# Xharlie/BtcDet

Hardware: AMD Instinct MI355X
Metric: scenes/s fwd+bwd KITTI-Car bs=2/GPU (BtcDet hot path) (higher is better)
Workload: dtype f32

## Files before the change

### btcdet_amd/_lib.py

```python
import ctypes
import os

import numpy as np
import torch

_HERE = os.path.dirname(os.path.abspath(__file__))
LIB_PATH = os.path.join(_HERE, "libbtcdet_hip.so")
_lib = None

c_i32p = ctypes.POINTER(ctypes.c_int32)
c_f32p = ctypes.POINTER(ctypes.c_float)
vp = ctypes.c_void_p
ci = ctypes.c_int
sz = ctypes.c_size_t

MODE_SUBM, MODE_CONV, MODE_TRANSPOSE = 0, 1, 2


class BtcHipError(RuntimeError):
    pass


class BtcOccConfig(ctypes.Structure):
    _fields_ = [("batch", ctypes.c_int32), ("grid", ctypes.c_int32 * 3), ("sphere_grid", ctypes.c_int32 * 3),
# ... 169 lines not shown

AUGMENT_EXPORTED_SYMBOLS = tuple(_AUGMENT_SIGS.keys())

_BESTMATCH_SIGS = {
    "btc_place_templates": (ci, [vp, ctypes.c_longlong, vp, vp, vp, vp, vp, ci, ci, vp, vp, ctypes.c_longlong, ci, vp, vp]),
}

BESTMATCH_EXPORTED_SYMBOLS = tuple(_BESTMATCH_SIGS.keys())

_FRAMES_SIGS = {
    "btc_fov_crop_ws_bytes": (sz, [ci, ci]),
    "btc_fov_crop": (ci, [vp, ci, ci, vp, ci, vp, ci, vp, vp, vp, vp, sz, vp]),
}

FRAMES_EXPORTED_SYMBOLS = tuple(_FRAMES_SIGS.keys())

_GTDB_SIGS = {
    "btc_cut_objects_ws_bytes": (sz, [ci, ci, ci, ci]),
    "btc_cut_objects": (ci, [vp, ci, ci, vp, ci, vp, vp, vp, ci, ci, ci, vp, vp, vp, vp, sz, vp]),
}

GTDB_EXPORTED_SYMBOLS = tuple(_GTDB_SIGS.keys())

cf = ctypes.c_float
_TEMPLATES_SIGS = {
    "btc_nn_sqdist": (ci, [vp, ci, vp, ci, vp, vp, ci, ci, vp, vp]),
    "btc_match_candidates": (ci, [vp, ci, vp, vp, ci, vp, vp, ci, ci, cf, cf, cf, ci, ci, vp, vp, vp]),
    "btc_select_templates_ws_bytes": (sz, [ci, ci, ci]),
    "btc_select_templates": (ci, [vp, ci, vp, ci, vp, vp, vp, vp, vp, vp, ci, ci, ci, ci, ci, cf, cf, cf, ci, ci, vp, vp, vp, vp, vp, sz, vp]),
}

TEMPLATES_EXPORTED_SYMBOLS = tuple(_TEMPLATES_SIGS.keys())


def lib():
    global _lib
    if _lib is None:
        if not os.path.exists(LIB_PATH):
            raise BtcHipError(
                f"{LIB_PATH} not found: build it with `python -c 'import __graft_entry__ as g; g.build()'` "
                f"or `make -C btcdet_amd/csrc` (there is no CPU fallback for the hot path)")
        L = ctypes.CDLL(LIB_PATH)
        for name, (res, args) in (list(_SIGS.items()) + list(_INFER_SIGS.items()) + list(_AUGMENT_SIGS.items()) + list(_BESTMATCH_SIGS.items()) +
                                  list(_FRAMES_SIGS.items()) + list(_GTDB_SIGS.items()) + list(_TEMPLATES_SIGS.items())):
            fn = getattr(L, name)
            fn.restype = res
            fn.argtypes = args
        for kv in filter(None, os.environ.get("BTC_TUNE", "").split(",")):
            k, v = kv.split("=")
            if L.btc_tune_set(int(k), int(v)) != 0:
                raise BtcHipError("BTC_TUNE: bad entry %r" % kv)
        _lib = L
    return _lib


_fast = False


def fast():
    global _fast
    if _fast is False:
        _fast = None
        if os.environ.get("BTC_FASTPATH", "1") != "0":
            try:
                lib()
                from . import _btcfast
                if _btcfast.abi_version() == lib().btc_version():
                    _fast = _btcfast
            except ImportError:
                _fast = None
    return _fast


def check(rc, what):
    if rc != 0:
        msg = lib().btc_last_error().decode("utf-8", "replace")
        raise BtcHipError(f"{what} failed (code {rc}): {msg}")
# ... 55 lines not shown
```

### btcdet_amd/csrc/binding.cpp

```cpp
#include <torch/extension.h>
#include <c10/hip/HIPCachingAllocator.h>
#include <c10/hip/HIPStream.h>
#include <c10/hip/HIPGuard.h>
#include <hip/hip_runtime_api.h>
#include <torch/csrc/autograd/engine.h>

#include <atomic>
#include <mutex>
#include <stdexcept>
#include <string>
#include <unordered_map>
#include <cstdio>
#include <cstdlib>
#include <memory>
#include <tuple>
#include <vector>

#include "../../include/btcdet_hip.h"
#include "../../include/btcdet_hip_infer.h"

namespace {

using at::Tensor;
using OptTensor = c10::optional<at::Tensor>;

inline void chk(int rc, const char* what) {
  if (rc != 0) throw std::runtime_error(std::string(what) + " failed (code " + std::to_string(rc) + "): " + btc_last_error());
}

inline const float* fptr(const OptTensor& t) { return (t.has_value() && t->defined()) ? (const float*)t->data_ptr() : nullptr; }
inline void* vptr(const OptTensor& t) { return (t.has_value() && t->defined()) ? t->data_ptr() : nullptr; }
inline void* st(int64_t stream) { return reinterpret_cast<void*>(stream); }
inline const int32_t* ip(int64_t p) { return reinterpret_cast<const int32_t*>(p); }


inline void need(bool ok, const char* msg) {
  if (!ok) throw std::runtime_error(msg);
}
inline void need(bool ok, const char* who, const char* msg) {
  if (!ok) throw std::runtime_error(std::string(who) + msg);
}

struct WqEntry {
  c10::weak_intrusive_ptr<c10::TensorImpl> weak;
  uint32_t version;
  Tensor q;
  WqEntry(c10::weak_intrusive_ptr<c10::TensorImpl> w, uint32_t v, Tensor t) : weak(std::move(w)), version(v), q(std::move(t)) {}
};
std::mutex g_wq_mu;
std::unordered_map<const void*, WqEntry> g_wq;
std::unordered_map<const void*, WqEntry> g_ws;

// ... 793 lines not shown
    }
    x = ConvBNReLUNode::apply(x, weights[i], biases[i], map_fwd[i], map_bwd[i], order_fwd[i], order_bwd[i], gammas[i], betas[i], rms[i], rvs[i], nbts[i], use_batch[i],
                              momenta[i], epss[i], relus[i], ws, ws_bytes[i], overlaps[i], allow_defers[i]);
  }
  return x;
}

void adam_group_step(const std::vector<Tensor>& params, const std::vector<Tensor>& grads, const Tensor& chunk_seg, const Tensor& chunk_off,
                     const Tensor& chunk_len, const Tensor& chunk_flat, const std::vector<int64_t>& seg_chunk0, const Tensor& flat_p,
                     const Tensor& flat_m, const Tensor& flat_v, int64_t step, double lr, double beta1, double beta2, double eps, double weight_decay,
                     double clip, const Tensor& ws, int64_t stream) {
  const size_t n = params.size();
  need(grads.size() == n && seg_chunk0.size() == n + 1, "adam_group_step: list lengths differ");
  std::vector<const float*> ptrs(n);
  std::vector<int32_t> sc(n + 1);
  for (size_t i = 0; i < n; ++i) {
    const Tensor& g = grads[i];
    need(g.defined() && g.is_contiguous() && g.scalar_type() == at::kFloat && g.numel() == params[i].numel() && g.get_device() == flat_p.get_device(),
         "adam_group_step: every gradient must be a contiguous fp32 tensor of its parameter's size on the parameters' device");
    ptrs[i] = (const float*)g.data_ptr();
    sc[i] = (int32_t)seg_chunk0[i];
  }
  sc[n] = (int32_t)seg_chunk0[n];
  chk(btc_adam_group_step(ptrs.data(), (int)n, (const int32_t*)chunk_seg.data_ptr(), (const int32_t*)chunk_off.data_ptr(),
                          (const int32_t*)chunk_len.data_ptr(), (const int64_t*)chunk_flat.data_ptr(), sc.data(), (int)chunk_seg.numel(),
                          (float*)flat_p.data_ptr(), (float*)flat_m.data_ptr(), (float*)flat_v.data_ptr(), (long long)step, (float)lr, (float)beta1,
                          (float)beta2, (float)eps, (float)weight_decay, (float)clip, ws.data_ptr(), (size_t)ws.numel(), st(stream)),
      "btc_adam_group_step");
  for (size_t i = 0; i < n; ++i) params[i].unsafeGetTensorImpl()->bump_version();
}

struct ParamList {
  std::vector<Tensor> p;
};

std::shared_ptr<ParamList> make_param_list(const std::vector<Tensor>& params) {
  auto pl = std::make_shared<ParamList>();
  pl->p = params;
  return pl;
}

bool adam_group_step_pl(const std::shared_ptr<ParamList>& pl, const Tensor& chunk_seg, const Tensor& chunk_off, const Tensor& chunk_len,
                        const Tensor& chunk_flat, const std::vector<int64_t>& seg_chunk0, const Tensor& flat_p, const Tensor& flat_m,
                        const Tensor& flat_v, int64_t step, double lr, double beta1, double beta2, double eps, double weight_decay, double clip,
                        const Tensor& ws, int64_t stream) {
  const size_t n = pl->p.size();
  std::vector<Tensor> grads(n);
  for (size_t i = 0; i < n; ++i) {
    const Tensor& g = pl->p[i].grad();
    if (!(g.defined() && g.is_contiguous() && g.scalar_type() == at::kFloat && g.numel() == pl->p[i].numel() && g.get_device() == flat_p.get_device()))
      return false;
    grads[i] = g;
  }
  adam_group_step(pl->p, grads, chunk_seg, chunk_off, chunk_len, chunk_flat, seg_chunk0, flat_p, flat_m, flat_v, step, lr, beta1, beta2, eps,
                  weight_decay, clip, ws, stream);
  return true;
}

void clear_grads_pl(const std::shared_ptr<ParamList>& pl) {
  for (Tensor& t : pl->p) t.mutable_grad().reset();
}

void pack_grads(const std::vector<Tensor>& grads, const Tensor& chunk_seg, const Tensor& chunk_off, const Tensor& chunk_len, const Tensor& chunk_flat,
                const std::vector<int64_t>& seg_chunk0, const std::vector<int64_t>& sizes, const Tensor& flat, int64_t stream) {
  const size_t n = grads.size();
  need(seg_chunk0.size() == n + 1 && sizes.size() == n, "pack_grads: list lengths differ");
  std::vector<const float*> ptrs(n);
  std::vector<int32_t> sc(n + 1);
  for (size_t i = 0; i < n; ++i) {
    const Tensor& g = grads[i];
    need(g.defined() && g.is_contiguous() && g.scalar_type() == at::kFloat && g.numel() == sizes[i] && g.get_device() == flat.get_device(),
         "pack_grads: every gradient must be a contiguous fp32 tensor of its parameter's size on the bucket's device");
    ptrs[i] = (const float*)g.data_ptr();
    sc[i] = (int32_t)seg_chunk0[i];
  }
  sc[n] = (int32_t)seg_chunk0[n];
  chk(btc_grads_pack(ptrs.data(), (int)n, (const int32_t*)chunk_seg.data_ptr(), (const int32_t*)chunk_off.data_ptr(), (const int32_t*)chunk_len.data_ptr(),
                     (const int64_t*)chunk_flat.data_ptr(), sc.data(), (float*)flat.data_ptr(), st(stream)), "btc_grads_pack");
}

}

PYBIND11_MODULE(TORCH_EXTENSION_NAME, m) {
  m.doc() = "compiled PyTorch binding of libbtcdet_hip.so's hot entry points";
  m.def("split_weights", &split_weights, py::call_guard<py::gil_scoped_release>());
  m.def("bf16_weights", &bf16_weights, py::call_guard<py::gil_scoped_release>());
  m.def("conv_fwd", &conv_fwd, py::call_guard<py::gil_scoped_release>());
  m.def("bn_fwd", &bn_fwd, py::call_guard<py::gil_scoped_release>());
  m.def("conv_bn_fwd", &conv_bn_fwd, py::call_guard<py::gil_scoped_release>());
  m.def("conv_bn_eval_fold", &conv_bn_eval_fold, py::call_guard<py::gil_scoped_release>());
  m.def("eval_fold_calls", &eval_fold_calls);
  m.def("bn_bwd", &bn_bwd, py::call_guard<py::gil_scoped_release>());
  m.def("conv_bwd", &conv_bwd, py::call_guard<py::gil_scoped_release>());
  m.def("conv_bn_relu", &conv_bn_relu, py::call_guard<py::gil_scoped_release>());
  m.def("row_orders", &row_orders, py::call_guard<py::gil_scoped_release>());
  m.def("geometry_walk", &geometry_walk, py::call_guard<py::gil_scoped_release>());
  py::class_<PendingWalk, std::shared_ptr<PendingWalk>>(m, "PendingWalk");
  m.def("geometry_walk_start", &geometry_walk_start, py::call_guard<py::gil_scoped_release>());
  m.def("geometry_walk_finish", &geometry_walk_finish, py::call_guard<py::gil_scoped_release>());
  m.def("conv_bn_relu_chain", &conv_bn_relu_chain, py::call_guard<py::gil_scoped_release>());
  m.def("pack_grads", &pack_grads, py::call_guard<py::gil_scoped_release>());
  m.def("adam_group_step", &adam_group_step, py::call_guard<py::gil_scoped_release>());
  py::class_<ParamList, std::shared_ptr<ParamList>>(m, "ParamList");
  m.def("make_param_list", &make_param_list);
  m.def("adam_group_step_pl", &adam_group_step_pl, py::call_guard<py::gil_scoped_release>());
  m.def("clear_grads_pl", &clear_grads_pl);
  m.def("join_wgrad", &join_wgrad, py::call_guard<py::gil_scoped_release>());
  m.def("set_defer_wgrad_join", &set_defer_wgrad_join);
  m.def("set_side_stream", &set_side_stream);
  m.def("rulebook_subm", &rulebook_subm, py::call_guard<py::gil_scoped_release>());
  m.def("rulebook_conv", &rulebook_conv, py::call_guard<py::gil_scoped_release>());
  m.def("abi_version", []() { return btc_version(); });
}
```

### btcdet_amd/csrc/optim.hip

```cpp
#include "btc_common.h"

namespace {

constexpr int OPT_CHUNK = 1024;

struct GradPtrs {
  const float* g[BTC_ADAM_MAX_SEGMENTS];
};

__global__ __launch_bounds__(256) void adam_sqnorm(GradPtrs ptrs, const int32_t* __restrict__ chunk_seg, const int32_t* __restrict__ chunk_off,
                                                   const int32_t* __restrict__ chunk_len, int chunk0, double* __restrict__ partial) {
  __shared__ double s_sum[4];
  const int c = chunk0 + blockIdx.x;
  const float* g = ptrs.g[chunk_seg[c]] + chunk_off[c];
  const int len = chunk_len[c];
  double acc = 0.0;
#pragma unroll
  for (int u = 0; u < OPT_CHUNK / 256; ++u) {
    const int e = u * 256 + threadIdx.x;
    if (e < len) {
      const float v = g[e];
      acc += (double)v * v;
    }
  }
#pragma unroll
  for (int d = 32; d > 0; d >>= 1) acc += __shfl_down(acc, d, 64);
  if ((threadIdx.x & 63) == 0) s_sum[threadIdx.x >> 6] = acc;
  __syncthreads();
  if (threadIdx.x == 0) partial[c] = (s_sum[0] + s_sum[1]) + (s_sum[2] + s_sum[3]);
}

__global__ __launch_bounds__(256) void adam_total(const double* __restrict__ partial, int n_chunks, double* __restrict__ total_sq) {
  __shared__ double s_sum[256];
// ... 7 lines not shown
    *total_sq = t;
  }
}

__global__ __launch_bounds__(256) void adam_apply(GradPtrs ptrs, const int32_t* __restrict__ chunk_seg, const int32_t* __restrict__ chunk_off,
                                                  const int32_t* __restrict__ chunk_len, const int64_t* __restrict__ chunk_flat, int chunk0,
                                                  const double* __restrict__ total_sq, float clip, float decay, float lr_over_bc1, float beta1,
                                                  float beta2, float inv_sqrt_bc2, float eps, float* __restrict__ p, float* __restrict__ m,
                                                  float* __restrict__ v) {
  const int c = chunk0 + blockIdx.x;
  const float* g = ptrs.g[chunk_seg[c]] + chunk_off[c];
  const int len = chunk_len[c];
  const int64_t base = chunk_flat[c];
  float inv_coef = 1.f;
  if (clip > 0.f) {
    const float norm = (float)sqrt(*total_sq);
    inv_coef = fmaxf((norm + 1e-6f) / clip, 1.f);
  }
#pragma unroll
  for (int u = 0; u < OPT_CHUNK / 256; ++u) {
    const int e = u * 256 + threadIdx.x;
    if (e < len) {
      const float gr = g[e] / inv_coef;
      float pv = p[base + e] * decay;
      float mv = m[base + e], vv = v[base + e];
      mv = mv + (1.f - beta1) * (gr - mv);
      vv = beta2 * vv + (1.f - beta2) * gr * gr;
      const float denom = sqrtf(vv) * inv_sqrt_bc2 + eps;
      pv -= lr_over_bc1 * mv / denom;
      p[base + e] = pv;
      m[base + e] = mv;
      v[base + e] = vv;
    }
  }
}

__global__ __launch_bounds__(256) void grads_pack(GradPtrs ptrs, const int32_t* __restrict__ chunk_seg, const int32_t* __restrict__ chunk_off,
                                                  const int32_t* __restrict__ chunk_len, const int64_t* __restrict__ chunk_flat, int chunk0,
                                                  float* __restrict__ flat) {
  const int c = chunk0 + blockIdx.x;
  const float* g = ptrs.g[chunk_seg[c]] + chunk_off[c];
  const int len = chunk_len[c];
  float* out = flat + chunk_flat[c];
#pragma unroll
  for (int u = 0; u < OPT_CHUNK / 256; ++u) {
    const int e = u * 256 + threadIdx.x;
    if (e < len) out[e] = g[e];
  }
}

}

extern "C" int btc_adam_max_segments(void) { return BTC_ADAM_MAX_SEGMENTS; }

extern "C" int btc_grads_pack(const float* const* grads, int n_seg, const int32_t* chunk_seg, const int32_t* chunk_off, const int32_t* chunk_len,
                              const int64_t* chunk_flat, const int32_t* seg_chunk0, float* flat, void* stream_) {
  hipStream_t stream = (hipStream_t)stream_;
  BTC_CHECK_ARG(n_seg >= 0, "btc_grads_pack: bad sizes");
  for (int s0 = 0; s0 < n_seg; s0 += BTC_ADAM_MAX_SEGMENTS) {
    const int s1 = s0 + BTC_ADAM_MAX_SEGMENTS < n_seg ? s0 + BTC_ADAM_MAX_SEGMENTS : n_seg;
    GradPtrs ptrs;
    for (int s = s0; s < s1; ++s) {
      BTC_CHECK_ARG(grads[s] != nullptr, "btc_grads_pack: gradient %d is NULL", s);
      ptrs.g[s - s0] = grads[s];
    }
    const int c0 = seg_chunk0[s0], c1 = seg_chunk0[s1];
// ... 12 lines not shown
                                   float weight_decay, float clip, void* ws, size_t ws_bytes, void* stream_) {
  hipStream_t stream = (hipStream_t)stream_;
  BTC_CHECK_ARG(n_seg >= 0 && n_chunks >= 0 && step >= 1, "btc_adam_group_step: bad sizes");
  if (n_seg == 0 || n_chunks == 0) return BTC_OK;
  BTC_CHECK_ARG(ws_bytes >= btc_adam_group_ws_bytes(n_chunks), "btc_adam_group_step: workspace too small");
  double* total_sq = (double*)ws;
  double* partial = (double*)((char*)ws + 256);
  const double bc1 = 1.0 - pow((double)beta1, (double)step), bc2 = 1.0 - pow((double)beta2, (double)step);
  for (int pass = 0; pass < 2; ++pass) {
    if (pass == 1 && clip > 0.f) {
      adam_total<<<1, 256, 0, stream>>>(partial, n_chunks, total_sq);
      BTC_LAUNCH_CHECK();
    }
    for (int s0 = 0; s0 < n_seg; s0 += BTC_ADAM_MAX_SEGMENTS) {
      const int s1 = s0 + BTC_ADAM_MAX_SEGMENTS < n_seg ? s0 + BTC_ADAM_MAX_SEGMENTS : n_seg;
      GradPtrs ptrs;
      for (int s = s0; s < s1; ++s) {
        BTC_CHECK_ARG(grads[s] != nullptr, "btc_adam_group_step: gradient %d is NULL", s);
        ptrs.g[s - s0] = grads[s];
      }
      const int c0 = seg_chunk0[s0], c1 = seg_chunk0[s1];
      if (c1 <= c0) continue;
      if (pass == 0) {
        if (clip > 0.f) adam_sqnorm<<<c1 - c0, 256, 0, stream>>>(ptrs, chunk_seg, chunk_off, chunk_len, c0, partial);
      } else {
        adam_apply<<<c1 - c0, 256, 0, stream>>>(ptrs, chunk_seg, chunk_off, chunk_len, chunk_flat, c0, total_sq, clip, 1.f - weight_decay * lr,
                                               (float)((double)lr / bc1), beta1, beta2, (float)(1.0 / sqrt(bc2)), eps, params, exp_avg, exp_avg_sq);
      }
      BTC_LAUNCH_CHECK();
    }
  }
  return BTC_OK;
}
```

### btcdet_amd/csrc/rulebook.hip

```cpp
#include "btc_common.h"

namespace {

constexpr int RB_T = 256;
constexpr int RB_BLK = 8;
constexpr int RB_CHUNK = 256;
constexpr int RB_MAX_JOBS = 17;

struct Level {
  unsigned* words;
  int32_t* bprefix;
  int32_t* cprefix;
  int shape[3];
  int vol;
  long long nblk;
};

__host__ __device__ __forceinline__ long long lvl_cell(const Level& L, int b, int z, int y, int x) {
  return (long long)b * L.vol + ((long long)z * L.shape[1] + y) * L.shape[2] + x;
}

__device__ __forceinline__ void cell_coords(const Level& L, long long cell, int* b, int* z, int* y, int* x) {
  const int hw = L.shape[1] * L.shape[2];
  const int bb = (int)(cell / L.vol);
// ... 997 lines not shown
      const int lw = markb_span(nw);
      rb_mark_b<<<btc_cdiv(nw, 1LL << lw), RB_T, 0, stream>>>(W.lv[li], W.lo[li].ncell, g, W.lv[lo], lw);
      BTC_LAUNCH_CHECK();
    }
    BTC_CHECK_ARG(S.n < BTC_CHAIN_MAX_LAYERS, "btc_chain_levels: too many levels");
    S.lv[S.n] = W.lv[lo];
    S.chunk_sums[S.n] = W.chunk_sums[lo];
    S.counter[S.n] = W.counters + lo;
    S.d_total[S.n] = d_counts + i;
    S.out_idx[S.n] = (int4*)out_indices[i];
    S.cap[S.n] = (long long)h_cap[i];
    S.nchunks[S.n] = W.lo[lo].nchunks;
    S.block0[S.n] = (int)scan_blocks;
    scan_blocks += W.lo[lo].nchunks;
    ++S.n;
  }
  if (S.n == 0) return BTC_OK;
  S.block0[S.n] = (int)scan_blocks;
  BTC_CHECK_ARG(scan_blocks < (1LL << 31), "btc_chain_levels: grids too large");
  rb_scan_all<<<(unsigned)scan_blocks, RB_T, 0, stream>>>(S);
  BTC_LAUNCH_CHECK();
  long long emit_blocks = 0;
  for (int q = 0; q < S.n; ++q) {
    S.block0[q] = (int)emit_blocks;
    emit_blocks += btc_cdiv(S.lv[q].nblk * RB_BLK, RB_T);
  }
  S.block0[S.n] = (int)emit_blocks;
  BTC_CHECK_ARG(emit_blocks < (1LL << 31), "btc_chain_levels: grids too large");
  rb_emit_all<<<(unsigned)emit_blocks, RB_T, 0, stream>>>(S);
  BTC_LAUNCH_CHECK();
  return BTC_OK;
}

extern "C" int btc_chain_maps(const int32_t* indices, int n0, int batch, const BtcChainLayer* layers, int n_layers, const int32_t* h_counts,
                              int32_t* const* out_indices, int32_t* const* nbr_out, int32_t* const* nbr_in, int32_t* const* first_out,
                              int32_t* const* first_in, void* ws, size_t ws_bytes, void* stream_) {
  hipStream_t stream = (hipStream_t)stream_;
  ChainPlan P;
  int rc = chain_plan(layers, n_layers, &P);
  if (rc) return rc;
  ChainWs W;
  rc = chain_ws(layers, P, batch, n0, ws, &W);
  if (rc) return rc;
  BTC_CHECK_ARG(ws_bytes >= W.total_bytes, "btc_chain_maps: workspace too small");
  int rows_of[BTC_CHAIN_MAX_LAYERS + 1];
  const int32_t* idx_of[BTC_CHAIN_MAX_LAYERS + 1];
  rows_of[0] = n0;
  idx_of[0] = indices;
  for (int lv = 1; lv < P.n_levels; ++lv) {
    rows_of[lv] = h_counts[P.producer[lv]];
    idx_of[lv] = out_indices[P.producer[lv]];
  }
  {
    char* run_begin = nullptr;
    size_t run_bytes = 0;
    for (int i = 0; i <= n_layers; ++i) {
      char* p = nullptr;
      size_t bytes = 0;
      if (i < n_layers && layers[i].kind == 1 && P.lvl_in[i] == 0 && h_counts[i] > 0) {
        p = (char*)nbr_out[i];
        bytes = (size_t)h_counts[i] * layers[i].k[0] * layers[i].k[1] * layers[i].k[2] * sizeof(int32_t);
      } else if (i < n_layers) {
        continue;
      }
      if (p && run_begin && p >= run_begin + run_bytes && (size_t)(p - (run_begin + run_bytes)) < 256) {
        run_bytes = (size_t)(p - run_begin) + bytes;
      } else {
        if (run_begin) BTC_HIP(hipMemsetAsync(run_begin, 0xFF, run_bytes, stream));
        run_begin = p;
        run_bytes = bytes;
      }
    }
  }
  Jobs jobs;
  jobs.count = 0;
  long long blocks = 0;
  auto flush = [&]() -> int {
    if (jobs.count == 0) return BTC_OK;
    rb_fill<<<(unsigned)blocks, RB_T, 0, stream>>>(jobs);
    BTC_LAUNCH_CHECK();
    jobs.count = 0;
    blocks = 0;
    return BTC_OK;
  };
  auto add = [&](int type, int n, const BtcGeom& g, const Level& lvl, int ranked, int sorted, const int32_t* idx, int32_t* map, int32_t* map2,
                 int32_t* first, int32_t* first2 = nullptr) -> int {
    if (n <= 0) return BTC_OK;
    const long long nb = btc_cdiv(n, RB_ROWS);
    if (jobs.count == RB_MAX_JOBS || blocks + nb > 0x7fffffffLL) {
      int rc2 = flush();
      if (rc2) return rc2;
    }
    jobs.j[jobs.count++] = make_job(type, n, blocks, g, lvl, ranked, sorted, idx, map, map2, first, first2, W.keys, W.vals, W.hash_cap);
    blocks += nb;
    return BTC_OK;
  };
  for (int i = 0; i < n_layers; ++i) {
    if (layers[i].kind > 1) continue;
    if (layers[i].kind == 0 && !nbr_out[i] && !nbr_in[i]) continue;
    BTC_CHECK_ARG(nbr_out[i] && (layers[i].kind == 0 || nbr_in[i]), "btc_chain_maps: layer %d: nbr_out (and, for a strided layer, nbr_in) required", i);
    const int li = P.lvl_in[i];
    const BtcGeom& g = P.g[i];
    if (layers[i].kind == 1) {
      const int lo = P.lvl_out[i];
      int32_t* keys2 = (li == 0 && first_out) ? first_out[i] : nullptr;
      if (keys2 && h_counts[i] > 0)
        BTC_HIP(hipMemsetAsync(keys2, 0x7F, (size_t)h_counts[i] * sizeof(int32_t), stream));
      rc = add(JOB_FWD, rows_of[li], g, W.lv[lo], 1, li != 0, idx_of[li], nbr_in[i], li == 0 ? nbr_out[i] : nullptr, first_in ? first_in[i] : nullptr, keys2);
      if (rc) return rc;
      if (li != 0) {
        rc = add(JOB_BWD, rows_of[lo], g, W.lv[li], 1, 1, idx_of[lo], nbr_out[i], nullptr, first_out ? first_out[i] : nullptr);
        if (rc) return rc;
      }
    } else if (li == 0) {
      LevelLayout l0;
      rc = level_layout(batch, layers[i].in_shape, &l0);
      if (rc) return rc;
      rc = add(JOB_SUBM, rows_of[li], g, make_level(l0, layers[i].in_shape, nullptr, nullptr, nullptr), 0, 0, idx_of[li], nbr_out[i], nbr_in[i], nullptr);
      if (rc) return rc;
    } else {
      rc = add(JOB_SUBM, rows_of[li], g, W.lv[li], 1, 1, idx_of[li], nbr_out[i], nbr_in[i], nullptr);
      if (rc) return rc;
    }
  }
  return flush();
}

extern "C" size_t btc_pairs_from_nbr_ws_bytes(int n_out, int K) {
  const long long cnt = (long long)K * (n_out + 1);
  return btc_align((size_t)cnt * sizeof(int32_t)) + btc_scan_ws_bytes(cnt);
}

extern "C" int btc_pairs_from_nbr(const int32_t* nbr_out, int n_out, int K, int n_in, int32_t* pairs, int32_t* pair_num, void* ws,
                                  size_t ws_bytes, void* stream_) {
  hipStream_t stream = (hipStream_t)stream_;
  BTC_CHECK_ARG(n_out >= 0 && K >= 1 && n_in >= 0, "btc_pairs_from_nbr: bad sizes");
  BTC_CHECK_ARG(ws_bytes >= btc_pairs_from_nbr_ws_bytes(n_out, K), "btc_pairs_from_nbr: workspace too small");
  if (n_in > 0) BTC_HIP(hipMemsetAsync(pairs, 0xFF, (size_t)2 * K * n_in * sizeof(int32_t), stream));
  const long long cnt = (long long)K * (n_out + 1);
  BtcCarver cv(ws);
// ... 11 lines not shown
```

### btcdet_amd/train_step.py

```python
import math

import os

import torch


class OneCycle(object):

    def __init__(self, total_step, lr_max, moms, div_factor, pct_start):
        self.total = int(total_step)
        self.turn = int(self.total * pct_start)
        self.lr_max = float(lr_max)
        self.lr_low = self.lr_max / float(div_factor)
        self.lr_end = self.lr_low / 1e4
        self.mom_hi, self.mom_lo = float(moms[0]), float(moms[1])

    @staticmethod
    def _cos(start, end, pct):
        return end + (start - end) / 2.0 * (math.cos(math.pi * pct) + 1.0)

    def initial(self):
        return self.lr_low, self.mom_hi

    def at(self, it):
# ... 104 lines not shown
    @property
    def iteration(self):
        return max(g["it"] for g in self.groups) if self.groups else 0

    @iteration.setter
    def iteration(self, value):
        for g in self.groups:
            g["it"] = int(value)

    def read_grads_from(self, view_of, present=None, missing=None):
        for g in self.groups:
            g["grad_views"] = [view_of(p) for p in g["params"]]
        self._present, self._missing = present, missing

    def zero_grad(self, set_to_none=True):
        for g in self.groups:
            pl = self._param_list(g)
            if pl is not None:
                g["flat"]["F"].clear_grads_pl(pl)
                continue
            for p in g["params"]:
                p.grad = None

    @staticmethod
    def _param_list(g):
        fl = g.get("flat")
        if fl is None or not hasattr(fl.get("F"), "make_param_list"):
            return None
        pl = fl.get("plist")
        if pl is None:
            pl = fl["plist"] = fl["F"].make_param_list(list(g["params"]))
        return pl

    def _flat_step_params(self, g):
        fl = g.get("flat")
        if fl is None or fl["n"] < 0:
            return False
        pl = self._param_list(g)
        if pl is None:
            return False
        from ._lib import stream_ptr
        if not fl["F"].adam_group_step_pl(pl, fl["seg"], fl["off"], fl["len"], fl["flat"], fl["seg0"], fl["p"], fl["m"], fl["v"], fl["n"] + 1,
                                          float(g["lr"]), float(g["mom"]), float(self.beta2), float(self.eps), float(g["weight_decay"]),
                                          float(g["clip"]), fl["ws"], stream_ptr()):
            return False
        fl["n"] += 1
        fl["synced"] = False
        return True

    def lrs(self):
        return [g["lr"] for g in self.groups]

    @torch.no_grad()
    def step(self, groups=None):
        last_norms = []
        for gi, g in enumerate(self.groups):
            if groups is not None and gi not in groups:
                continue
            params = g["params"]
            if params and "grad_views" not in g and self._flat_step_params(g):
                if g["clip"] > 0:
                    last_norms.append(g["flat"]["ws"][:8].view(torch.float64))
                nlr, nmom = g["sched"].at(g["it"])
                g["lr"], g["mom"] = max(nlr, g["lr_clip"]), nmom
                g["it"] += 1
                continue
            if "grad_views" in g:
                grads = g["grad_views"]
                if self._present is None or (self._missing is not None and not self._missing()):
                    keep = params
                else:
                    keep = [i for i, p in enumerate(params) if self._present(p)]
            else:
                grads = [p.grad for p in params]
                keep = [i for i, gr in enumerate(grads) if gr is not None]
            if params and "flat" in g and self._flat_step(g, grads if len(keep) == len(params) else [None]):
                if g["clip"] > 0:
                    last_norms.append(g["flat"]["ws"][:8].view(torch.float64))
                nlr, nmom = g["sched"].at(g["it"])
                g["lr"], g["mom"] = max(nlr, g["lr_clip"]), nmom
                g["it"] += 1
                continue
            if len(keep) != len(params):
                params, grads = [params[i] for i in keep], [grads[i] for i in keep]
                ea, es, st = [g["exp_avgs"][i] for i in keep], [g["exp_avg_sqs"][i] for i in keep], [g["steps"][i] for i in keep]
            else:
                ea, es, st = g["exp_avgs"], g["exp_avg_sqs"], g["steps"]
            if not params:
                nlr, nmom = g["sched"].at(g["it"])
                g["lr"], g["mom"] = max(nlr, g["lr_clip"]), nmom
                g["it"] += 1
                continue
# ... 54 lines not shown
```

### btcdet_amd/trainer.py

```python
import os
import threading

import torch


_SUMSQ_WS = {}


class MeanSquare2(torch.autograd.Function):

    @staticmethod
    def forward(ctx, a, scale_a, b, scale_b):
        ka = float(scale_a) / max(a.numel(), 1)
        kb = float(scale_b) / max(b.numel(), 1) if b is not None else 0.0
        ctx.k = (ka, kb)
        ok = lambda t: t is None or (t.is_cuda and t.dtype in (torch.float32, torch.bfloat16))
        if not (ok(a) and ok(b)):
            ctx.save_for_backward(a, b)
            ctx.fused = False
            out = torch.linalg.vector_norm(a.reshape(-1), dtype=torch.float32) ** 2 * ka
            return out if b is None else out + torch.linalg.vector_norm(b.reshape(-1), dtype=torch.float32) ** 2 * kb
        from ._lib import check, lib, ptr, stream_ptr
        a = a.contiguous()
        b = b.contiguous() if b is not None else None
# ... 46 lines not shown
            one = _ONES[key] = torch.ones(t.shape, dtype=t.dtype, device=t.device)
        seeds.append(one)
    torch.autograd.backward((loss,) + more, seeds)


def make_step(model, ddp, proc, opts, grad_sync=None, prefetch_stream=None, threaded=True, det_stream=None, opt_stream=None,
              det_loss=None, pipeline=None):
    from . import affinity as _aff
    from .spconv import ops as _ops
    det_loss = det_loss or stand_in_det_loss
    pipeline_wanted = pipeline is None or bool(pipeline)
    _placed = [0]

    def _place_threads():
        if _placed[0] < 16:
            _placed[0] += 1
            if _placed[0] <= 3 or _placed[0] == 16:
                _aff.place_thread("train")
                _aff.place_other_threads()
    pending = {}
    pool = None
    if (prefetch_stream is not None and threaded) or det_stream is not None:
        from concurrent.futures import ThreadPoolExecutor
        pool = ThreadPoolExecutor(max_workers=1, initializer=_aff.place_thread, initargs=("occupancy" if pipeline_wanted else "prepare",))
    device = next(model.parameters()).device
    split_backward = grad_sync is not None and ddp is model and len(grad_sync.buckets) > 1 and getattr(grad_sync, "split_backward", False)
    bucket_of = getattr(grad_sync, "bucket_of", None) if grad_sync is not None else None

    _split = {}

    def refresh_planes(group):
        if "lists" not in _split:
            _split["lists"] = split_weight_lists(model) if hasattr(model, "occ_modules") else ((None, ()), (None, ()))
        kind, ws = _split["lists"][group]
        if ws:
            from .spconv import ops as _o
            from ._lib import stream_ptr
            (_o.fast().bf16_weights if kind == "bf16" else _o.fast().split_weights)(ws, stream_ptr())

    def prep(next_batch):
        torch.cuda.set_device(device)
        if timing is None:
            return model.prepare(next_batch, stream=prefetch_stream)
        import time
        t0, c0 = time.perf_counter(), time.thread_time()
        out = model.prepare(next_batch, stream=prefetch_stream)
        timing["p_prepare"] = timing.get("p_prepare", 0.0) + time.perf_counter() - t0
        timing["cpu_prep"] = timing.get("cpu_prep", 0.0) + time.thread_time() - c0
        return out

    def occ_backward(loss):
        torch.cuda.set_device(device)
        _backward(loss)

    if pipeline is None:
        pipeline = True
    pipeline = bool(pipeline and det_stream is not None and ddp is model and (grad_sync is None or bucket_of is not None)
                    and prefetch_stream is not None and threaded and len(opts) == 1 and hasattr(opts[0], "groups") and len(opts[0].groups) == 2)
    ahead_occ = {}

    def _put(slot, batch, value):
        slot.clear()
        slot["batch"], slot["value"] = batch, value

    def _take(slot, batch):
        hit = slot.get("value") if slot.get("batch") is batch else None
        slot.clear()
        return hit
# ... 333 lines not shown
```

Measured before the change: 589.6.

## Fuse bf16/split weight-plane refresh into Adam step and batch rulebook prefills

The Adam apply kernel now also writes the quantized bf16 or three-way split weight planes, in both normal and transposed layouts, straight from the updated parameters. A tiled shared-memory path handles the transpose. This removes the separate refresh_planes pass that re-read every weight after each optimizer step. The grad-norm reduction becomes a single-kernel last-arriver total. Separately, the per-layer hipMemsetAsync calls in chain_maps are replaced by one multi-job fill kernel that also handles the first_out prefill, with its pattern changed from 0x7F bytes to BTC_EMPTY_IDX, which risks a semantic mismatch.

```diff
diff --git a/btcdet_amd/_lib.py b/btcdet_amd/_lib.py
--- a/btcdet_amd/_lib.py
+++ b/btcdet_amd/_lib.py
@@ -225,6 +225,12 @@
 
 TEMPLATES_EXPORTED_SYMBOLS = tuple(_TEMPLATES_SIGS.keys())
 
+_OPTIM_SIGS = {
+    "btc_adam_group_step_planes": (ci, [vp, ci, vp, vp, vp, vp, c_i32p, ci, vp, vp, vp, ctypes.c_longlong, cf, cf, cf, cf, cf, cf, vp, ci, vp, sz, vp]),
+}
+
+OPTIM_EXPORTED_SYMBOLS = tuple(_OPTIM_SIGS.keys())
+
 
 def lib():
     global _lib
@@ -235,7 +241,7 @@
                 f"or `make -C btcdet_amd/csrc` (there is no CPU fallback for the hot path)")
         L = ctypes.CDLL(LIB_PATH)
         for name, (res, args) in (list(_SIGS.items()) + list(_INFER_SIGS.items()) + list(_AUGMENT_SIGS.items()) + list(_BESTMATCH_SIGS.items()) +
-                                  list(_FRAMES_SIGS.items()) + list(_GTDB_SIGS.items()) + list(_TEMPLATES_SIGS.items())):
+                                  list(_FRAMES_SIGS.items()) + list(_GTDB_SIGS.items()) + list(_TEMPLATES_SIGS.items()) + list(_OPTIM_SIGS.items())):
             fn = getattr(L, name)
             fn.restype = res
             fn.argtypes = args
diff --git a/btcdet_amd/csrc/binding.cpp b/btcdet_amd/csrc/binding.cpp
--- a/btcdet_amd/csrc/binding.cpp
+++ b/btcdet_amd/csrc/binding.cpp
@@ -18,6 +18,7 @@
 
 #include "../../include/btcdet_hip.h"
 #include "../../include/btcdet_hip_infer.h"
+#include "../../include/btcdet_hip_optim.h"
 
 namespace {
 
@@ -877,6 +878,9 @@
 
 struct ParamList {
   std::vector<Tensor> p;
+  int planes = 0;
+  Tensor plane_table;
+  std::vector<std::pair<Tensor, Tensor>> plane_w;
 };
 
 std::shared_ptr<ParamList> make_param_list(const std::vector<Tensor>& params) {
@@ -884,21 +888,79 @@
   pl->p = params;
   return pl;
 }
+
+bool param_list_set_planes(const std::shared_ptr<ParamList>& pl, const std::vector<Tensor>& weights, int64_t planes, int64_t stream) {
+  need(planes == 1 || planes == 3, "param_list_set_planes: planes must be 1 or 3");
+  pl->planes = 0;
+  pl->plane_w.clear();
+  pl->plane_table = Tensor();
+  if (weights.empty() || pl->p.empty()) return false;
+  std::unordered_map<const void*, size_t> index;
+  for (size_t i = 0; i < pl->p.size(); ++i) index.emplace(pl->p[i].unsafeGetTensorImpl(), i);
+  for (const Tensor& w : weights)
+    if (index.find(w.unsafeGetTensorImpl()) == index.end()) return false;
+  refresh_weights(weights, stream, (int)planes);
+  Tensor host = at::zeros({(int64_t)(pl->p.size() * sizeof(BtcAdamPlanes))}, at::TensorOptions().dtype(at::kByte));
+  BtcAdamPlanes* tab = (BtcAdamPlanes*)host.data_ptr();
+  {
+    std::lock_guard<std::mutex> lock(g_wq_mu);
+    auto& cache = planes == 1 ? g_wq : g_ws;
+    for (const Tensor& w : weights) {
+      const Tensor& q = cache.find(w.unsafeGetTensorImpl())->second.q;
+      const int64_t cin = w.size(-2), cout = w.size(-1);
+      BtcAdamPlanes& e = tab[index[w.unsafeGetTensorImpl()]];
+      e.w = q.data_ptr();
+      e.wt = (char*)q.data_ptr() + 2 * planes * w.numel();
+      e.K = (int32_t)(w.numel() / (cin * cout)); e.Cin = (int32_t)cin; e.Cout = (int32_t)cout;
+      pl->plane_w.emplace_back(w, q);
+    }
+  }
+  pl->plane_table = host.to(pl->p[0].device());
+  pl->planes = (int)planes;
+  return true;
+}
+
+std::vector<std::pair<Tensor, Tensor>> param_list_planes(const std::shared_ptr<ParamList>& pl) { return pl->plane_w; }
 
 bool adam_group_step_pl(const std::shared_ptr<ParamList>& pl, const Tensor& chunk_seg, const Tensor& chunk_off, const Tensor& chunk_len,
                         const Tensor& chunk_flat, const std::vector<int64_t>& seg_chunk0, const Tensor& flat_p, const Tensor& flat_m,
                         const Tensor& flat_v, int64_t step, double lr, double beta1, double beta2, double eps, double weight_decay, double clip,
                         const Tensor& ws, int64_t stream) {
   const size_t n = pl->p.size();
-  std::vector<Tensor> grads(n);
+  need(seg_chunk0.size() == n + 1, "adam_group_step_pl: list lengths differ");
+  std::vector<const float*> ptrs(n);
+  std::vector<int32_t> sc(n + 1);
   for (size_t i = 0; i < n; ++i) {
     const Tensor& g = pl->p[i].grad();
     if (!(g.defined() && g.is_contiguous() && g.scalar_type() == at::kFloat && g.numel() == pl->p[i].numel() && g.get_device() == flat_p.get_device()))
       return false;
-    grads[i] = g;
-  }
-  adam_group_step(pl->p, grads, chunk_seg, chunk_off, chunk_len, chunk_flat, seg_chunk0, flat_p, flat_m, flat_v, step, lr, beta1, beta2, eps,
-                  weight_decay, clip, ws, stream);
+    ptrs[i] = (const float*)g.data_ptr();
+    sc[i] = (int32_t)seg_chunk0[i];
+  }
+  sc[n] = (int32_t)seg_chunk0[n];
+  chk(btc_adam_group_step_planes(ptrs.data(), (int)n, (const int32_t*)chunk_seg.data_ptr(), (const int32_t*)chunk_off.data_ptr(),
+                                 (const int32_t*)chunk_len.data_ptr(), (const int64_t*)chunk_flat.data_ptr(), sc.data(), (int)chunk_seg.numel(),
+                                 (float*)flat_p.data_ptr(), (float*)flat_m.data_ptr(), (float*)flat_v.data_ptr(), (long long)step, (float)lr,
+                                 (float)beta1, (float)beta2, (float)eps, (float)weight_decay, (float)clip,
+                                 pl->planes ? (const BtcAdamPlanes*)pl->plane_table.data_ptr() : nullptr, pl->planes, ws.data_ptr(),
+                                 (size_t)ws.numel(), st(stream)),
+      "btc_adam_group_step_planes");
+  for (size_t i = 0; i < n; ++i) pl->p[i].unsafeGetTensorImpl()->bump_version();
+  if (pl->planes) {
+    std::lock_guard<std::mutex> lock(g_wq_mu);
+    auto& cache = pl->planes == 1 ? g_wq : g_ws;
+    for (auto& wq : pl->plane_w) {
+      const Tensor& w = wq.first;
+      const void* key = w.unsafeGetTensorImpl();
+      auto it = cache.find(key);
+      if (it != cache.end() && !it->second.weak.expired() && it->second.q.data_ptr() == wq.second.data_ptr()) {
+        it->second.version = (uint32_t)w._version();
+        continue;
+      }
+      if (it != cache.end()) cache.erase(it);
+      cache.emplace(key, WqEntry(c10::weak_intrusive_ptr<c10::TensorImpl>(w.getIntrusivePtr()), (uint32_t)w._version(), wq.second));
+    }
+  }
   return true;
 }
 
@@ -949,6 +1011,8 @@
   py::class_<ParamList, std::shared_ptr<ParamList>>(m, "ParamList");
   m.def("make_param_list", &make_param_list);
   m.def("adam_group_step_pl", &adam_group_step_pl, py::call_guard<py::gil_scoped_release>());
+  m.def("param_list_set_planes", &param_list_set_planes, py::call_guard<py::gil_scoped_release>());
+  m.def("param_list_planes", &param_list_planes);
   m.def("clear_grads_pl", &clear_grads_pl);
   m.def("join_wgrad", &join_wgrad, py::call_guard<py::gil_scoped_release>());
   m.def("set_defer_wgrad_join", &set_defer_wgrad_join);
diff --git a/btcdet_amd/csrc/optim.hip b/btcdet_amd/csrc/optim.hip
--- a/btcdet_amd/csrc/optim.hip
+++ b/btcdet_amd/csrc/optim.hip
@@ -1,4 +1,6 @@
 #include "btc_common.h"
+#include "conv_tile.h"
+#include "../../include/btcdet_hip_optim.h"
 
 namespace {
 
@@ -72,6 +74,140 @@
       m[base + e] = mv;
       v[base + e] = vv;
     }
+  }
+}
+
+constexpr int OPT_COUNTER_BYTE = 64;
+
+constexpr int OPT_NORM_GROUPS = 512;
+
+__global__ __launch_bounds__(256) void adam_sqnorm_total(GradPtrs ptrs, const int32_t* __restrict__ chunk_seg, const int32_t* __restrict__ chunk_off,
+                                                         const int32_t* __restrict__ chunk_len, int chunk0, int chunk1, int n_chunks, int n_groups,
+                                                         double* __restrict__ partial, int32_t* __restrict__ counter, double* __restrict__ total_sq) {
+  __shared__ double s_sum[256];
+  constexpr int U = OPT_CHUNK / 256;
+  float x[U], y[U];
+  auto load = [&](int c, float (&d)[U]) {
+    const float* g = ptrs.g[chunk_seg[c]] + chunk_off[c];
+    const int len = chunk_len[c];
+#pragma unroll
+    for (int u = 0; u < U; ++u) {
+      const int e = u * 256 + threadIdx.x;
+      d[u] = e < len ? g[e] : 0.f;
+    }
+  };
+  int c = chunk0 + blockIdx.x;
+  load(c, x);
+  for (int it = 0;; ++it) {
+    const int cn = c + (int)gridDim.x;
+    if (cn < chunk1) load(cn, y);
+    double acc = 0.0;
+#pragma unroll
+    for (int u = 0; u < U; ++u) acc += (double)x[u] * x[u];
+#pragma unroll
+    for (int d = 32; d > 0; d >>= 1) acc += __shfl_down(acc, d, 64);
+    double* s = s_sum + (it & 1) * 4;
+    if ((threadIdx.x & 63) == 0) s[threadIdx.x >> 6] = acc;
+    __syncthreads();
+    if (threadIdx.x == 0) btc_st_agent(&partial[c], (s[0] + s[1]) + (s[2] + s[3]));
+    if (cn >= chunk1) break;
+    c = cn;
+#pragma unroll
+    for (int u = 0; u < U; ++u) x[u] = y[u];
+  }
+  if (!btc_last_arriver(counter, n_groups)) return;
+  double acc = 0.0;
+  for (int i = threadIdx.x; i < n_chunks; i += 256) acc += btc_ld_agent(&partial[i]);
+  s_sum[threadIdx.x] = acc;
+  __syncthreads();
+  if (threadIdx.x == 0) {
+    double t = 0.0;
+    for (int i = 0; i < 256; ++i) t += s_sum[i];
+    *total_sq = t;
+    btc_st_agent(counter, (int32_t)0);
+  }
+}
+
+template <int PLANES>
+__global__ __launch_bounds__(256) void adam_apply_planes(GradPtrs ptrs, const int32_t* __restrict__ chunk_seg, const int32_t* __restrict__ chunk_off,
+                                                         const int32_t* __restrict__ chunk_len, const int64_t* __restrict__ chunk_flat, int chunk0,
+                                                         const double* __restrict__ total_sq, float clip, float decay, float lr_over_bc1, float beta1,
+                                                         float beta2, float inv_sqrt_bc2, float eps, float* __restrict__ p, float* __restrict__ m,
+                                                         float* __restrict__ v, const BtcAdamPlanes* __restrict__ seg_planes, int seg0) {
+  __shared__ uint2 s_q[PLANES][OPT_CHUNK / 4];
+  const int c = chunk0 + blockIdx.x;
+  const int seg = chunk_seg[c], off = chunk_off[c];
+  const float* g = ptrs.g[seg] + off;
+  const int len = chunk_len[c];
+  const int64_t base = chunk_flat[c];
+  const BtcAdamPlanes pl = seg_planes[seg0 + seg];
+  unsigned short* const w_q = (unsigned short*)pl.w;
+  unsigned short* const wt_q = (unsigned short*)pl.wt;
+  const unsigned Cin = (unsigned)pl.Cin, Cout = (unsigned)pl.Cout;
+  const long long per = (long long)Cin * Cout, n = (long long)pl.K * per;
+  const unsigned per32 = per < 0x80000000LL ? (unsigned)per : 0x80000000u;
+  const unsigned R = Cout ? OPT_CHUNK / Cout : 0;
+  const bool tile = w_q != nullptr && len == OPT_CHUNK && R >= 4 && (R & 3) == 0 && R * Cout == OPT_CHUNK && Cin % R == 0 &&
+                    (long long)off + OPT_CHUNK <= n && (((uintptr_t)w_q | (uintptr_t)wt_q) & 7) == 0;
+  float inv_coef = 1.f;
+  if (clip > 0.f) {
+    const float norm = (float)sqrt(*total_sq);
+    inv_coef = fmaxf((norm + 1e-6f) / clip, 1.f);
+  }
+#pragma unroll
+  for (int u = 0; u < OPT_CHUNK / 256; ++u) {
+    const int e = u * 256 + threadIdx.x;
+    if (e < len) {
+      const float gr = g[e] / inv_coef;
+      float pv = p[base + e] * decay;
+      float mv = m[base + e], vv = v[base + e];
+      mv = mv + (1.f - beta1) * (gr - mv);
+      vv = beta2 * vv + (1.f - beta2) * gr * gr;
+      const float denom = sqrtf(vv) * inv_sqrt_bc2 + eps;
+      pv -= lr_over_bc1 * mv / denom;
+      p[base + e] = pv;
+      m[base + e] = mv;
+      v[base + e] = vv;
+      if (w_q == nullptr) continue;
+      unsigned short q[PLANES];
+      if (PLANES == 3) {
+        const BtcSplit3 x = btc_split3(pv);
+        q[0] = (unsigned short)(x.hi >> 16); q[PLANES / 2] = (unsigned short)(x.mid >> 16); q[PLANES - 1] = (unsigned short)(x.lo >> 16);
+      } else {
+        q[0] = btc_f32_to_bf16(pv);
+      }
+      if (tile) {
+#pragma unroll
+        for (int j = 0; j < PLANES; ++j) ((unsigned short*)s_q[j])[e] = q[j];
+        continue;
+      }
+      const unsigned i = (unsigned)off + (unsigned)e;
+      if ((long long)i < n) {
+        const unsigned k = i / per32, rem = i - k * per32;
+        const unsigned ci = rem / Cout, co = rem - ci * Cout;
+        const long long it = (long long)k * per + (long long)co * Cin + ci;
+#pragma unroll
+        for (int j = 0; j < PLANES; ++j) {
+          w_q[j * n + i] = q[j];
+          wt_q[j * n + it] = q[j];
+        }
+      }
+    }
+  }
+  if (!tile) return;
+  __syncthreads();
+  const unsigned t = threadIdx.x;
+  const unsigned row0 = (unsigned)off / Cout, k = row0 / Cin, ci0 = row0 - k * Cin;
+  const unsigned co = t / (R / 4), quad = t % (R / 4);
+  const long long dst_w = (long long)off + 4 * t, dst_wt = (long long)k * per + (long long)co * Cin + ci0 + 4 * quad;
+#pragma unroll
+  for (int j = 0; j < PLANES; ++j) {
+    *reinterpret_cast<uint2*>(w_q + j * n + dst_w) = s_q[j][t];
+    const unsigned short* sq = (const unsigned short*)s_q[j] + (4 * quad) * Cout + co;
+    uint2 o;
+    o.x = (unsigned)sq[0] | ((unsigned)sq[Cout] << 16);
+    o.y = (unsigned)sq[2 * Cout] | ((unsigned)sq[3 * Cout] << 16);
+    *reinterpret_cast<uint2*>(wt_q + j * n + dst_wt) = o;
   }
 }
 
@@ -150,3 +286,52 @@
   }
   return BTC_OK;
 }
+
+extern "C" int btc_adam_group_step_planes(const float* const* grads, int n_seg, const int32_t* chunk_seg, const int32_t* chunk_off,
+                                          const int32_t* chunk_len, const int64_t* chunk_flat, const int32_t* seg_chunk0, int n_chunks,
+                                          float* params, float* exp_avg, float* exp_avg_sq, long long step, float lr, float beta1, float beta2,
+                                          float eps, float weight_decay, float clip, const BtcAdamPlanes* seg_planes, int planes, void* ws,
+                                          size_t ws_bytes, void* stream_) {
+  hipStream_t stream = (hipStream_t)stream_;
+  BTC_CHECK_ARG(n_seg >= 0 && n_chunks >= 0 && step >= 1, "btc_adam_group_step_planes: bad sizes");
+  BTC_CHECK_ARG(planes == 0 || planes == 1 || planes == 3, "btc_adam_group_step_planes: planes must be 0, 1 or 3");
+  if (n_seg == 0 || n_chunks == 0) return BTC_OK;
+  BTC_CHECK_ARG(ws_bytes >= btc_adam_group_ws_bytes(n_chunks), "btc_adam_group_step_planes: workspace too small");
+  for (int s = 0; s < n_seg; ++s) BTC_CHECK_ARG(grads[s] != nullptr, "btc_adam_group_step_planes: gradient %d is NULL", s);
+  BTC_CHECK_ARG(seg_chunk0[0] == 0 && seg_chunk0[n_seg] == n_chunks, "btc_adam_group_step_planes: seg_chunk0 does not span the n_chunks chunks");
+  if (seg_planes == nullptr) planes = 0;
+  double* total_sq = (double*)ws;
+  int32_t* counter = (int32_t*)((char*)ws + OPT_COUNTER_BYTE);
+  double* partial = (double*)((char*)ws + 256);
+  const double bc1 = 1.0 - pow((double)beta1, (double)step), bc2 = 1.0 - pow((double)beta2, (double)step);
+  const float decay = 1.f - weight_decay * lr, lr_over_bc1 = (float)((double)lr / bc1), inv_sqrt_bc2 = (float)(1.0 / sqrt(bc2));
+  int n_groups = 0;
+  for (int s0 = 0; s0 < n_seg; s0 += BTC_ADAM_MAX_SEGMENTS) {
+    const int s1 = s0 + BTC_ADAM_MAX_SEGMENTS < n_seg ? s0 + BTC_ADAM_MAX_SEGMENTS : n_seg;
+    const int nc = seg_chunk0[s1] - seg_chunk0[s0];
+    n_groups += nc < OPT_NORM_GROUPS ? (nc > 0 ? nc : 0) : OPT_NORM_GROUPS;
+  }
+  for (int pass = clip > 0.f ? 0 : 1; pass < 2; ++pass) {
+    for (int s0 = 0; s0 < n_seg; s0 += BTC_ADAM_MAX_SEGMENTS) {
+      const int s1 = s0 + BTC_ADAM_MAX_SEGMENTS < n_seg ? s0 + BTC_ADAM_MAX_SEGMENTS : n_seg;
+      GradPtrs ptrs;
+      for (int s = s0; s < s1; ++s) ptrs.g[s - s0] = grads[s];
+      const int c0 = seg_chunk0[s0], c1 = seg_chunk0[s1];
+      if (c1 <= c0) continue;
+      if (pass == 0)
+        adam_sqnorm_total<<<c1 - c0 < OPT_NORM_GROUPS ? c1 - c0 : OPT_NORM_GROUPS, 256, 0, stream>>>(ptrs, chunk_seg, chunk_off, chunk_len, c0, c1, n_chunks,
+                                                                                                   n_groups, partial, counter, total_sq);
+      else if (planes == 3)
+        adam_apply_planes<3><<<c1 - c0, 256, 0, stream>>>(ptrs, chunk_seg, chunk_off, chunk_len, chunk_flat, c0, total_sq, clip, decay, lr_over_bc1,
+                                                          beta1, beta2, inv_sqrt_bc2, eps, params, exp_avg, exp_avg_sq, seg_planes, s0);
+      else if (planes == 1)
+        adam_apply_planes<1><<<c1 - c0, 256, 0, stream>>>(ptrs, chunk_seg, chunk_off, chunk_len, chunk_flat, c0, total_sq, clip, decay, lr_over_bc1,
+                                                          beta1, beta2, inv_sqrt_bc2, eps, params, exp_avg, exp_avg_sq, seg_planes, s0);
+      else
+        adam_apply<<<c1 - c0, 256, 0, stream>>>(ptrs, chunk_seg, chunk_off, chunk_len, chunk_flat, c0, total_sq, clip, decay, lr_over_bc1, beta1,
+                                                beta2, inv_sqrt_bc2, eps, params, exp_avg, exp_avg_sq);
+      BTC_LAUNCH_CHECK();
+    }
+  }
+  return BTC_OK;
+}
diff --git a/btcdet_amd/csrc/rulebook.hip b/btcdet_amd/csrc/rulebook.hip
--- a/btcdet_amd/csrc/rulebook.hip
+++ b/btcdet_amd/csrc/rulebook.hip
@@ -1053,6 +1053,72 @@
   return BTC_OK;
 }
 
+namespace {
+
+constexpr int FILL_MAX = 16;
+constexpr int FILL_BLOCK = 4096;
+struct FillJobs {
+  uint32_t* p[FILL_MAX];
+  unsigned long long ndw[FILL_MAX];
+  uint32_t pattern[FILL_MAX];
+  int first_block[FILL_MAX + 1];
+  int n;
+};
+
+__global__ __launch_bounds__(256) void prefill_multi(const FillJobs f) {
+  int s = 0;
+  while (s + 1 < f.n && (int)blockIdx.x >= f.first_block[s + 1]) ++s;
+  uint32_t* p = f.p[s];
+  const unsigned long long ndw = f.ndw[s];
+  const uint32_t v = f.pattern[s];
+  const bool aligned = ((uintptr_t)p & 15) == 0;
+  const unsigned long long b0 = (unsigned long long)((int)blockIdx.x - f.first_block[s]) * FILL_BLOCK;
+#pragma unroll
+  for (int u = 0; u < FILL_BLOCK / 1024; ++u) {
+    const unsigned long long i = b0 + (unsigned long long)u * 1024 + 4 * threadIdx.x;
+    if (aligned && i + 4 <= ndw) {
+      *reinterpret_cast<uint4*>(p + i) = make_uint4(v, v, v, v);
+    } else {
+#pragma unroll
+      for (int x = 0; x < 4; ++x)
+        if (i + x < ndw) p[i + x] = v;
+    }
+  }
+}
+
+struct Prefill {
+  FillJobs f;
+  long long blocks = 0;
+  hipStream_t stream;
+  explicit Prefill(hipStream_t s) : stream(s) { f.n = 0; }
+  int flush() {
+    if (f.n == 0) return BTC_OK;
+    f.first_block[f.n] = (int)blocks;
+    prefill_multi<<<(unsigned)blocks, 256, 0, stream>>>(f);
+    BTC_LAUNCH_CHECK();
+    f.n = 0;
+    blocks = 0;
+    return BTC_OK;
+  }
+  int add(void* p, size_t bytes, uint32_t pattern) {
+    if (!p || bytes < 4) return BTC_OK;
+    const long long nb = (long long)((bytes / 4 + FILL_BLOCK - 1) / FILL_BLOCK);
+    if (f.n == FILL_MAX || blocks + nb > 0x7fffffffLL) {
+      int rc = flush();
+      if (rc) return rc;
+    }
+    f.p[f.n] = (uint32_t*)p;
+    f.ndw[f.n] = bytes / 4;
+    f.pattern[f.n] = pattern;
+    f.first_block[f.n] = (int)blocks;
+    ++f.n;
+    blocks += nb;
+    return BTC_OK;
+  }
+};
+
+}
+
 extern "C" int btc_chain_maps(const int32_t* indices, int n0, int batch, const BtcChainLayer* layers, int n_layers, const int32_t* h_counts,
                               int32_t* const* out_indices, int32_t* const* nbr_out, int32_t* const* nbr_in, int32_t* const* first_out,
                               int32_t* const* first_in, void* ws, size_t ws_bytes, void* stream_) {
@@ -1073,25 +1139,18 @@
     idx_of[lv] = out_indices[P.producer[lv]];
   }
   {
-    char* run_begin = nullptr;
-    size_t run_bytes = 0;
-    for (int i = 0; i <= n_layers; ++i) {
-      char* p = nullptr;
-      size_t bytes = 0;
-      if (i < n_layers && layers[i].kind == 1 && P.lvl_in[i] == 0 && h_counts[i] > 0) {
-        p = (char*)nbr_out[i];
-        bytes = (size_t)h_counts[i] * layers[i].k[0] * layers[i].k[1] * layers[i].k[2] * sizeof(int32_t);
-      } else if (i < n_layers) {
-        continue;
+    Prefill pre(stream);
+    for (int i = 0; i < n_layers; ++i) {
+      if (!(layers[i].kind == 1 && P.lvl_in[i] == 0 && h_counts[i] > 0)) continue;
+      rc = pre.add(nbr_out[i], (size_t)h_counts[i] * layers[i].k[0] * layers[i].k[1] * layers[i].k[2] * sizeof(int32_t), 0xFFFFFFFFu);
+      if (rc) return rc;
+      if (first_out && first_out[i]) {
+        rc = pre.add(first_out[i], (size_t)h_counts[i] * sizeof(int32_t), (uint32_t)BTC_EMPTY_IDX);
+        if (rc) return rc;
       }
-      if (p && run_begin && p >= run_begin + run_bytes && (size_t)(p - (run_begin + run_bytes)) < 256) {
-        run_bytes = (size_t)(p - run_begin) + bytes;
-      } else {
-        if (run_begin) BTC_HIP(hipMemsetAsync(run_begin, 0xFF, run_bytes, stream));
-        run_begin = p;
-        run_bytes = bytes;
-      }
-    }
+    }
+    rc = pre.flush();
+    if (rc) return rc;
   }
   Jobs jobs;
   jobs.count = 0;
@@ -1125,8 +1184,6 @@
     if (layers[i].kind == 1) {
       const int lo = P.lvl_out[i];
       int32_t* keys2 = (li == 0 && first_out) ? first_out[i] : nullptr;
-      if (keys2 && h_counts[i] > 0)
-        BTC_HIP(hipMemsetAsync(keys2, 0x7F, (size_t)h_counts[i] * sizeof(int32_t), stream));
       rc = add(JOB_FWD, rows_of[li], g, W.lv[lo], 1, li != 0, idx_of[li], nbr_in[i], li == 0 ? nbr_out[i] : nullptr, first_in ? first_in[i] : nullptr, keys2);
       if (rc) return rc;
       if (li != 0) {
diff --git a/btcdet_amd/train_step.py b/btcdet_amd/train_step.py
--- a/btcdet_amd/train_step.py
+++ b/btcdet_amd/train_step.py
@@ -160,6 +160,20 @@
             pl = fl["plist"] = fl["F"].make_param_list(list(g["params"]))
         return pl
 
+    def attach_planes(self, gi, kind, weights):
+        g = self.groups[gi]
+        pl = self._param_list(g)
+        if pl is None or not weights or not hasattr(g["flat"]["F"], "param_list_set_planes"):
+            return False
+        from ._lib import stream_ptr
+        g["flat"]["planes"] = 3 if kind == "split" else 1
+        g["flat"]["planes_on"] = bool(g["flat"]["F"].param_list_set_planes(pl, list(weights), g["flat"]["planes"], stream_ptr()))
+        return g["flat"]["planes_on"]
+
+    def planes_written(self, gi):
+        fl = self.groups[gi].get("flat")
+        return bool(fl is not None and fl.get("planes_fresh"))
+
     def _flat_step_params(self, g):
         fl = g.get("flat")
         if fl is None or fl["n"] < 0:
@@ -174,6 +188,13 @@
             return False
         fl["n"] += 1
         fl["synced"] = False
+        if fl.get("planes_on"):
+            fl["planes_fresh"] = True
+            from .spconv import ops
+            if ops.PROFILE is not None:
+                import weakref
+                for w, q in fl["F"].param_list_planes(pl):
+                    ops._WQ[(id(w), fl["planes"])] = (weakref.ref(w), w._version, q)
         return True
 
     def lrs(self):
@@ -186,6 +207,8 @@
             if groups is not None and gi not in groups:
                 continue
             params = g["params"]
+            if "flat" in g:
+                g["flat"]["planes_fresh"] = False
             if params and "grad_views" not in g and self._flat_step_params(g):
                 if g["clip"] > 0:
                     last_norms.append(g["flat"]["ws"][:8].view(torch.float64))
diff --git a/btcdet_amd/trainer.py b/btcdet_amd/trainer.py
--- a/btcdet_amd/trainer.py
+++ b/btcdet_amd/trainer.py
@@ -102,8 +102,17 @@
     def refresh_planes(group):
         if "lists" not in _split:
             _split["lists"] = split_weight_lists(model) if hasattr(model, "occ_modules") else ((None, ()), (None, ()))
+            _split["attached"] = [False, False]
         kind, ws = _split["lists"][group]
         if ws:
+            opt = opts[0]
+            if _split["attached"][group]:
+                if opt.planes_written(group):
+                    return
+            elif _split["attached"][group] is False and len(opts) == 1 and hasattr(opt, "attach_planes") and len(getattr(opt, "groups", ())) == 2:
+                _split["attached"][group] = True if opt.attach_planes(group, kind, ws) else None
+                if _split["attached"][group]:
+                    return
             from .spconv import ops as _o
             from ._lib import stream_ptr
             (_o.fast().bf16_weights if kind == "bf16" else _o.fast().split_weights)(ws, stream_ptr())
diff --git a/include/btcdet_hip_optim.h b/include/btcdet_hip_optim.h
--- /dev/null
+++ b/include/btcdet_hip_optim.h
@@ -0,0 +1,29 @@
+#ifndef BTCDET_HIP_OPTIM_H
+#define BTCDET_HIP_OPTIM_H
+
+#include <stddef.h>
+#include <stdint.h>
+
+#include "btcdet_hip.h"
+
+#ifdef __cplusplus
+extern "C" {
+#endif
+
+typedef struct BtcAdamPlanes {
+  void* w;
+  void* wt;
+  int32_t K, Cin, Cout;
+  int32_t reserved;
+} BtcAdamPlanes;
+
+int btc_adam_group_step_planes(const float* const* grads, int n_seg, const int32_t* chunk_seg, const int32_t* chunk_off,
+                               const int32_t* chunk_len, const int64_t* chunk_flat, const int32_t* seg_chunk0, int n_chunks,
+                               float* params, float* exp_avg, float* exp_avg_sq, long long step, float lr, float beta1, float beta2,
+                               float eps, float weight_decay, float clip, const BtcAdamPlanes* seg_planes, int planes, void* ws,
+                               size_t ws_bytes, void* stream);
+
+#ifdef __cplusplus
+}
+#endif
+#endif
```

New measurement: 591.3 (median of 6 runs). About the same (+0.3%).
